# mbilos/stribor

Measured on NVIDIA B200. Metric: log_prob samples/s, 8-layer spline coupling d=64, higher is better.
Workload: dtype f32

## Files before the change

stribor_b200/csrc/tc_layer.cu:

```cuda
#include "common.cuh"
#include "stb_math.cuh"
#include "tc_common.cuh"
#include "tc_pack.cuh"
#include "tc_spline16.cuh"

namespace stb {
using namespace tc;

namespace tcl {
using namespace sp16;

constexpr int kHid = 64;
constexpr int kK1 = 32;
constexpr int kPPad = 48;
constexpr int kG = 2;
constexpr int kChunkN = kG * kPPad;
constexpr int kMaxDim = 64;
constexpr int kMaxTr = 32;
constexpr int kMaxChunks = kMaxTr / kG;
constexpr int kTileRows = 256;
constexpr int kXsStride = kMaxDim + 1;
constexpr int kStages = 3;
constexpr int kMaxChain = 8;
constexpr int kEpiPerSub = 2;
constexpr int kEpiWarps = 2 * 4 * kEpiPerSub;
constexpr int kEpiWarp0 = 3;
constexpr int kThreads = (kEpiWarp0 + kEpiWarps) * 32;
constexpr int kEpiThreads = kEpiWarps * 32;

constexpr uint32_t kMagic = 0x53544232u;
struct Header {
    uint32_t magic;
    int32_t kind, dim, n_cond, n_tr, n_chunks, P, act;
    float s2;
    uint32_t maxbits;
    int32_t cond_idx[kK1];
    int32_t tr_idx[kMaxTr];
    uint32_t noshift_mask;
    int32_t n_lat;
    int32_t n_bins;
    int32_t pad[256 - 13 - kK1 - kMaxTr];
};
static_assert(sizeof(Header) == 1024, "header layout");
constexpr uint32_t kOffB1 = 1024;
constexpr uint32_t kOffB2 = kOffB1 + kHid * 4;
constexpr uint32_t kSmallBytes = kOffB2 + kMaxChunks * kChunkN * 4;
constexpr uint32_t kOffW1 = 8192;
constexpr uint32_t kW1Part = kHid * kK1 * 2;
constexpr uint32_t kW1Bytes = 3 * kW1Part;
constexpr uint32_t kA1Part = 128 * kK1 * 2;
constexpr uint32_t kOffW2 = kOffW1 + kW1Bytes;
constexpr uint32_t kChunkBytes = 2 * kChunkN * kHid * 2;
constexpr uint32_t kPackedBytes = kOffW2 + kMaxChunks * kChunkBytes;
constexpr uint32_t kHeadBytes = kOffW1 + kW1Bytes;
static_assert(kHeadBytes <= kChunkBytes, "the layer head fits a ring stage");

constexpr uint32_t kSmXs = 0;
constexpr uint32_t kSmA = kSmXs + kTileRows * kXsStride * 4;
constexpr uint32_t kABytes = 32768;
constexpr uint32_t kSmW1 = kSmA + 2 * kABytes;
constexpr uint32_t kSmB = kSmW1 + kW1Bytes;
constexpr uint32_t kSmSmall = kSmB + kStages * kChunkBytes;
constexpr uint32_t kSmBar = (kSmSmall + kSmallBytes + 15) & ~15u;
constexpr uint32_t kSmLd = kSmBar + 256;
constexpr uint32_t kSmemBytes = kSmLd + (kEpiPerSub - 1) * kTileRows * 4;
static_assert(kSmemBytes <= 227 * 1024, "shared memory budget");
static_assert(kSmA % 16 == 0 && kSmW1 % 16 == 0 && kSmB % 16 == 0 && kSmSmall % 16 == 0, "alignment");

struct Bars {
    uint64_t acc_full[2][2], acc_empty[2][2];
    uint64_t setup;
    uint64_t b_full[kStages], b_empty[kStages];
    uint64_t a1_ready[2], acc1_full[2], h_ready[2];
};
static_assert(sizeof(Bars) <= 256, "barrier block");

constexpr uint32_t kColAcc1 = 0;
constexpr uint32_t kColAcc2 = 128;
constexpr uint32_t kTmemCols = 512;

struct Args {
    const uint8_t* packed;
    const float* x;
    float* y;
    float* ldj;
    int ldj_mode;
    int base_log_prob;
    int inverse;
    float lower, upper;
    long long rows;
    int n_tiles;
    int n_layers, dim;
    const uint8_t* chain_packed[kMaxChain];
    float lower_l[kMaxChain], upper_l[kMaxChain];
    int n_chunks_l[kMaxChain];
    const float* latent;
    int lat_stride;
    int32_t* bins;
    int permuted;
    ChainPerm perm;
};

template <int KIND, bool INVERSE, bool CHAIN, bool BINS = false>
__global__ void __launch_bounds__(kThreads, 1) tc_spline_layer_kernel(const Args A) {
    extern __shared__ __align__(1024) uint8_t smem[];
    float* xs = reinterpret_cast<float*>(smem + kSmXs);
    uint8_t* abuf = smem + kSmA;
    uint8_t* w1s = smem + kSmW1;
    uint8_t* bst = smem + kSmB;
    const Header* hdr = reinterpret_cast<const Header*>(smem + kSmSmall);
    const float* b1s = reinterpret_cast<const float*>(smem + kSmSmall + kOffB1);
    const float* b2s = reinterpret_cast<const float*>(smem + kSmSmall + kOffB2);
    Bars* bars = reinterpret_cast<Bars*>(smem + kSmBar);
    float* ld_s = reinterpret_cast<float*>(smem + kSmLd);

    const int tid = threadIdx.x, warp = tid >> 5, lane = tid & 31;

    if (tid == 0) {
        mbar_init(&bars->setup, 1);
        for (int i = 0; i < kStages; ++i) { mbar_init(&bars->b_full[i], 1); mbar_init(&bars->b_empty[i], 2); }
        for (int s = 0; s < 2; ++s) {
            mbar_init(&bars->a1_ready[s], kEpiWarps);
            mbar_init(&bars->acc1_full[s], 1);
            mbar_init(&bars->h_ready[s], kEpiWarps);
            for (int b = 0; b < 2; ++b) { mbar_init(&bars->acc_full[s][b], 1); mbar_init(&bars->acc_empty[s][b], 8); }
        }
        fence_mbar_init();
    }
    __shared__ uint32_t tmem_base_s;
    if (warp == 1) tmem_alloc(&tmem_base_s, kTmemCols);
    tc_fence_before();
    __syncthreads();
    tc_fence_after();
    const uint32_t tmem = tmem_base_s;

    if (!CHAIN) {
        if (tid == 0) {
            mbar_arrive_expect_tx(&bars->setup, kSmallBytes + kW1Bytes);
            bulk_g2s(smem + kSmSmall, A.packed, kSmallBytes, &bars->setup);
            bulk_g2s(w1s, A.packed + kOffW1, kW1Bytes, &bars->setup);
        }
        mbar_wait(&bars->setup, 0);
    }

    const int n_layers = CHAIN ? A.n_layers : 1;
    const int d = CHAIN ? A.dim : hdr->dim;
    int n_tr = CHAIN ? 0 : hdr->n_tr, n_cond = CHAIN ? 0 : hdr->n_cond, n_chunks = CHAIN ? 0 : hdr->n_chunks;
    int n_lat = CHAIN ? 0 : hdr->n_lat;
    int act = CHAIN ? 0 : hdr->act;
    float s2 = CHAIN ? 1.f : hdr->s2;
    float s2l = s2 * 1.4426950408889634f;
    const int dshift = ((d & (d - 1)) == 0) ? (31 - __clz(d)) : -1;
    const int my_tiles = (A.n_tiles > (int)blockIdx.x) ? (A.n_tiles - 1 - (int)blockIdx.x) / (int)gridDim.x + 1 : 0;

    if (warp == 0) {
        if (lane == 0) {
            uint32_t cc = 0;
            for (int it = 0; it < my_tiles; ++it) {
                if (it + 1 < my_tiles) {
                    const long long nrow0 = ((long long)blockIdx.x + (long long)(it + 1) * gridDim.x) * kTileRows;
                    const long long nb = min((long long)kTileRows, A.rows - nrow0) * d * 4;
                    const char* src = reinterpret_cast<const char*>(A.x + nrow0 * d);
                    if (nb >= 16 && ((reinterpret_cast<uintptr_t>(src) & 15) == 0))
                        asm volatile("cp.async.bulk.prefetch.L2.global [%0], %1;" ::"l"(src), "r"((uint32_t)(nb & ~15LL)) : "memory");
                }
                for (int l = 0; l < n_layers; ++l) {
                    const uint8_t* img = CHAIN ? A.chain_packed[l] : A.packed;
                    const int nch = CHAIN ? A.n_chunks_l[l] : n_chunks;
                    if (CHAIN) {
                        const uint32_t st = cc % kStages, use = cc / kStages;
                        mbar_wait_relaxed(&bars->b_empty[st], (use & 1) ^ 1);
                        mbar_arrive_expect_tx(&bars->b_full[st], kHeadBytes);
                        bulk_g2s(bst + st * kChunkBytes, img, kHeadBytes, &bars->b_full[st]);
                        ++cc;
                    }
                    for (int c = 0; c < nch; ++c, ++cc) {
                        const uint32_t st = cc % kStages, use = cc / kStages;
                        mbar_wait_relaxed(&bars->b_empty[st], (use & 1) ^ 1);
                        mbar_arrive_expect_tx(&bars->b_full[st], kChunkBytes);
                        bulk_g2s(bst + st * kChunkBytes, img + kOffW2 + (size_t)c * kChunkBytes, kChunkBytes,
                                 &bars->b_full[st]);
                    }
                }
            }
        }
    } else if (warp < kEpiWarp0) {
        if (lane == 0) {
            const int s = warp - 1;
            const uint32_t idesc1 = make_idesc(FMT_BF16, 128, kHid);
            const uint32_t idesc2 = make_idesc(FMT_F16, 128, kChunkN);
            uint32_t cc = 0;
            uint32_t rc = 0;
            uint32_t hp = 0;
            for (int it = 0; it < my_tiles; ++it)
            for (int l = 0; l < n_layers; ++l, ++hp) {
                const uint32_t tpar = hp & 1;
                const int nch = CHAIN ? A.n_chunks_l[l] : n_chunks;
                {
                    uint32_t b0 = smem_u32(w1s);
                    const uint32_t hst = rc % kStages;
                    if (CHAIN) {
                        mbar_wait_relaxed(&bars->b_full[hst], (rc / kStages) & 1);
                        b0 = smem_u32(bst + hst * kChunkBytes) + kOffW1;
                    }
                    mbar_wait_relaxed(&bars->a1_ready[s], tpar);
                    tc_fence_after();
                    const uint32_t a0 = smem_u32(abuf + s * kABytes);
                    const uint32_t dcol = tmem + kColAcc1 + s * kHid;
                    uint32_t acc = 0;
#pragma unroll
                    for (int p = 0; p < 8; ++p) {
                        const int pa = (p == 0 || p == 3 || p == 6) ? 1 : ((p == 1 || p == 4) ? 2 : 0);
                        const int pb = (p == 0 || p == 2) ? 2 : ((p == 1 || p == 3 || p == 5) ? 1 : 0);
#pragma unroll
                        for (int ks = 0; ks < kK1 / 16; ++ks) {
                            umma_f16(dcol, make_smem_desc(a0 + pa * kA1Part + ks * 256, 128, 512),
                                     make_smem_desc(b0 + pb * kW1Part + ks * 256, 128, 512), idesc1, acc);
                            acc = 1;
                        }
                    }
                    umma_commit(&bars->acc1_full[s]);
                    if (CHAIN) { umma_commit(&bars->b_empty[hst]); ++rc; }
                }
                for (int c = 0; c < nch; ++c, ++cc, ++rc) {
                    const uint32_t st = rc % kStages, use = rc / kStages;
                    mbar_wait_relaxed(&bars->b_full[st], use & 1);
                    const uint32_t buf = cc & 1, buse = cc >> 1;
                    if (c == 0) mbar_wait_relaxed(&bars->h_ready[s], tpar);
                    mbar_wait_relaxed(&bars->acc_empty[s][buf], (buse & 1) ^ 1);
                    tc_fence_after();
                    const uint32_t a_hi = smem_u32(abuf + s * kABytes), a_lo = a_hi + 16384;
                    const uint32_t b_hi = smem_u32(bst + st * kChunkBytes), b_lo = b_hi + 12288;
                    const uint32_t dcol = tmem + kColAcc2 + (s * 2 + buf) * kChunkN;
                    uint32_t acc = 0;
#pragma unroll
                    for (int p = 0; p < 3; ++p) {
                        const uint32_t aa = (p == 0) ? a_lo : a_hi, bb = (p == 1) ? b_lo : b_hi;
#pragma unroll
                        for (int ks = 0; ks < kHid / 16; ++ks) {
                            umma_f16(dcol, make_smem_desc(aa + ks * 256, 128, 1024),
                                     make_smem_desc(bb + ks * 256, 128, 1024), idesc2, acc);
                            acc = 1;
                        }
                    }
                    umma_commit(&bars->acc_full[s][buf]);
                    umma_commit(&bars->b_empty[st]);
                }
            }
        }
    } else if (warp >= kEpiWarp0) {
        const int q = warp & 3;
        const int cls = (warp - (kEpiWarp0 + ((q - kEpiWarp0) & 3))) >> 2;
        const int s = cls & 1, r3 = cls >> 1;
        const int etid = tid - kEpiWarp0 * 32;
        const int rloc = q * 32 + lane;
        const int rt = s * 128 + rloc;
        float* xrow = xs + rt * kXsStride;
        const uint32_t a_row_off = (uint32_t)(rloc >> 3) * 1024 + (uint32_t)(rloc & 7) * 16;
        const uint32_t lane_sel = (uint32_t)(q * 32) << 16;
        const bool want_ld = A.ldj_mode != STB_LDJ_NONE;
        float lo = A.lower, hi = A.upper;
        float inv_span = 1.f / (hi - lo);
        const uint32_t full_bar = pin(smem_u32(&bars->acc_full[s][0]));
        const uint32_t empty_bar = pin(smem_u32(&bars->acc_empty[s][0]));
        const uint32_t col_base = pin(tmem + lane_sel + kColAcc2 + (uint32_t)(s * 2) * kChunkN);
        const uint32_t tr_idx_a = pin(smem_u32(&hdr->tr_idx[0]));
        const uint32_t b2_a = pin(smem_u32(b2s));
        const uint32_t xrow_a = pin(smem_u32(xrow));
        uint32_t noshift_mask = CHAIN ? 0u : hdr->noshift_mask;
        uint32_t cc = 0, rc = 0, hp = 0;

        for (int it = 0; it < my_tiles; ++it) {
            const long long tile = (long long)blockIdx.x + (long long)it * gridDim.x;
            const long long row0 = tile * kTileRows;
            const int nrows = (int)min((long long)kTileRows, A.rows - row0);

            {
                const float* xg = A.x + row0 * d;
                const int n = nrows * d;
                if ((d & 3) == 0 && ((reinterpret_cast<uintptr_t>(xg) & 15) == 0)) {
                    const int n4 = (kTileRows * d) >> 2;
                    for (int i0 = etid; i0 < n4; i0 += kEpiThreads * 4) {
                        float4 v[4];
#pragma unroll
                        for (int u = 0; u < 4; ++u) {
                            const int i = i0 + u * kEpiThreads;
                            v[u] = (i < n4 && i * 4 < n) ? __ldg(reinterpret_cast<const float4*>(xg) + i)
                                                         : make_float4(0.f, 0.f, 0.f, 0.f);
                        }
#pragma unroll
                        for (int u = 0; u < 4; ++u) {
                            const int i = i0 + u * kEpiThreads;
                            if (i < n4) {
                                const int r = (dshift >= 0) ? ((i * 4) >> dshift) : (i * 4) / d, c = (i * 4) - r * d;
                                float* dst = xs + r * kXsStride + c;
                                dst[0] = v[u].x; dst[1] = v[u].y; dst[2] = v[u].z; dst[3] = v[u].w;
                            }
                        }
                    }
                } else {
                    for (int i = etid; i < kTileRows * d; i += kEpiThreads) {
                        const int r = i / d, c = i - r * d;
                        xs[r * kXsStride + c] = (i < n) ? __ldg(xg + i) : 0.f;
                    }
                }
            }
            named_bar_sync(1, kEpiThreads);
            float ld_acc = 0.f;
#pragma unroll 1
            for (int l = 0; l < n_layers; ++l, ++hp) {
            const uint32_t tpar = hp & 1;
            if (CHAIN) {
                const uint32_t hst = rc % kStages;
                mbar_wait(&bars->b_full[hst], (rc / kStages) & 1);
                const uint4* src = reinterpret_cast<const uint4*>(bst + hst * kChunkBytes);
                uint4* dst = reinterpret_cast<uint4*>(smem + kSmSmall);
                for (int i = etid; i < (int)(kSmallBytes / 16); i += kEpiThreads) dst[i] = src[i];
                named_bar_sync(1, kEpiThreads);
                if (A.permuted) {
                    Header* h = const_cast<Header*>(hdr);
                    if (etid < kK1) { if (etid < h->n_cond) h->cond_idx[etid] = A.perm.phys[l][h->cond_idx[etid]]; }
                    else if (etid < kK1 + kMaxTr) h->tr_idx[etid - kK1] = A.perm.phys[l][h->tr_idx[etid - kK1]];
                    named_bar_sync(1, kEpiThreads);
                }
                n_tr = hdr->n_tr; n_cond = hdr->n_cond; n_chunks = hdr->n_chunks; act = hdr->act;
                n_lat = hdr->n_lat;
                s2 = hdr->s2; s2l = s2 * 1.4426950408889634f;
                noshift_mask = hdr->noshift_mask;
                lo = A.lower_l[l]; hi = A.upper_l[l]; inv_span = 1.f / (hi - lo);
                asm volatile("" : "+f"(lo), "+f"(hi), "+f"(inv_span));
                rc += 1u + (uint32_t)n_chunks;
            }

#pragma unroll 1
            for (int sp = 0; sp < 2; ++sp) {
                const float* xr = xs + (sp * 128 + rloc) * kXsStride;
                uint8_t* a_p = abuf + sp * kABytes;
                const uint32_t a1_row_off = (uint32_t)(rloc >> 3) * 512 + (uint32_t)(rloc & 7) * 16;
#pragma unroll 1
                for (int kc = cls; kc < kK1 / 8; kc += 2 * kEpiPerSub) {
                    __align__(16) __nv_bfloat16 q0[8], q1[8], q2[8];
#pragma unroll
                    for (int u = 0; u < 8; ++u) {
                        const int k = kc * 8 + u;
                        float v = 0.f;
                        if (k < n_cond) v = xr[hdr->cond_idx[k]];
                        else if (k < n_cond + n_lat && sp * 128 + rloc < nrows)
                            v = __ldg(A.latent + (row0 + sp * 128 + rloc) * A.lat_stride + (k - n_cond));
                        split_bf16x3(v, q0[u], q1[u], q2[u]);
                    }
                    *reinterpret_cast<uint4*>(a_p + a1_row_off + kc * 128) = *reinterpret_cast<const uint4*>(q0);
                    *reinterpret_cast<uint4*>(a_p + kA1Part + a1_row_off + kc * 128) = *reinterpret_cast<const uint4*>(q1);
                    *reinterpret_cast<uint4*>(a_p + 2 * kA1Part + a1_row_off + kc * 128) = *reinterpret_cast<const uint4*>(q2);
                }
                fence_proxy_async_smem();
                __syncwarp();
                if (lane == 0) mbar_arrive(&bars->a1_ready[sp]);
            }
#pragma unroll 1
            for (int sp = 0; sp < 2; ++sp) {
                uint8_t* a_p = abuf + sp * kABytes;
                mbar_wait(&bars->acc1_full[sp], tpar);
                tc_fence_after();
#pragma unroll 1
                for (int kc = cls; kc < kHid / 8; kc += 2 * kEpiPerSub) {
                    const int c0 = kc * 8;
                    float v[8];
                    tmem_ld8(tmem + lane_sel + kColAcc1 + sp * kHid + c0, v);
                    tmem_ld_wait();
                    __align__(16) __half hh[8], hl[8];
                    if (act == STB_ACT_TANH) {
#pragma unroll
                        for (int i = 0; i < 8; ++i) split_f16(tanh_fast(v[i] + b1s[c0 + i]), hh[i], hl[i]);
                    } else {
#pragma unroll
                        for (int i = 0; i < 8; ++i) v[i] = sigmoid_act(v[i] + b1s[c0 + i]);
#pragma unroll
                        for (int i = 0; i < 8; ++i) split_f16(v[i], hh[i], hl[i]);
                    }
                    *reinterpret_cast<uint4*>(a_p + a_row_off + kc * 128) = *reinterpret_cast<const uint4*>(hh);
                    *reinterpret_cast<uint4*>(a_p + 16384 + a_row_off + kc * 128) = *reinterpret_cast<const uint4*>(hl);
                }
                tc_fence_before();
                fence_proxy_async_smem();
                __syncwarp();
                if (lane == 0) mbar_arrive(&bars->h_ready[sp]);
            }

#pragma unroll 1
            for (int ji = r3; ji < kG * n_chunks; ji += kEpiPerSub) {
                const uint32_t ccc = cc + (uint32_t)(ji >> 1);
                const uint32_t buf = ccc & 1, buse = ccc >> 1;
                const int g = ji & 1;
                uint32_t j4;
                asm volatile("ld.shared.u32 %0, [%1];" : "=r"(j4) : "r"(tr_idx_a + 4u * (uint32_t)(ji < n_tr ? ji : 0)));
                j4 <<= 2;
                float xv;
                asm volatile("ld.shared.f32 %0, [%1];" : "=f"(xv) : "r"(xrow_a + j4));
                const bool inside = (ji < n_tr) && (xv >= lo) && (xv <= hi);
                const float* bb = b2s + ji * kPPad;
                mbar_wait_a(full_bar + buf * 8, buse & 1);
                tc_fence_after();
                const uint32_t col0 = col_base + buf * kChunkN + (uint32_t)g * kPPad;
                float out = xv, ld = 0.f;
                const bool shift = !((noshift_mask >> (ji & 31)) & 1u);
                const float2* bb2 = reinterpret_cast<const float2*>(bb);
                if (KIND == STB_RQS) {
                    RqsLoc loc;
                    {
                        float2 t[kBins];
                        tmem_ld16(col0, reinterpret_cast<float*>(t));
                        tmem_ld16(col0 + 16, reinterpret_cast<float*>(t) + 16);
                        tmem_ld_wait();
#pragma unroll
                        for (int i = 0; i < kBins; ++i) t[i] = __ffma2_rn(t[i], f2(s2l), bb2[i]);
                        loc = rqs16_locate<INVERSE>(t, shift, lo, inv_span, xv);
                    }
                    float dd[16];
                    tmem_ld16(col0 + 2 * kBins, dd);
                    tmem_ld_wait();
                    tc_fence_before();
                    __syncwarp();
                    if (lane == 0) mbar_arrive_a(empty_bar + buf * 8);
                    if (inside) {
                        float r0, r1;
                        pick_pair16(dd, loc.k, r0, r1);
                        const float u0 = (loc.k == 0) ? STB_RQS_EDGE_CONST : fmaf(r0, s2, bb[2 * kBins + loc.k - 1]);
                        const float u1 = (loc.k == kBins - 1) ? STB_RQS_EDGE_CONST : fmaf(r1, s2, bb[2 * kBins + loc.k]);
                        rqs16_finish<INVERSE>(loc, u0, u1, lo, hi, want_ld, xv, out, ld);
                    }
                    if (BINS && ji < n_tr && rt < nrows) A.bins[(row0 + rt) * d + (j4 >> 2)] = inside ? loc.k : -1;
                } else {
                    const float span = hi - lo;
                    const float u = (xv - lo) / span;
                    CubSel sel;
                    {
                        float2 t[kBins];
                        tmem_ld16(col0, reinterpret_cast<float*>(t));
                        tmem_ld16(col0 + 16, reinterpret_cast<float*>(t) + 16);
                        tmem_ld_wait();
#pragma unroll
                        for (int i = 0; i < kBins; ++i) t[i] = __ffma2_rn(t[i], f2(s2l), bb2[i]);
                        sel = cubic16_locate<INVERSE>(t, shift, u);
                    }
                    float dd[8];
                    tmem_ld8(col0 + 2 * kBins, dd);
                    tmem_ld_wait();
                    tc_fence_before();
                    __syncwarp();
                    if (lane == 0) mbar_arrive_a(empty_bar + buf * 8);
                    if (inside) {
                        const float ul = fmaf(dd[0], s2, bb[2 * kBins]), ur = fmaf(dd[1], s2, bb[2 * kBins + 1]);
                        cubic16_finish<INVERSE>(sel, ul, ur, lo, hi, want_ld, u, out, ld);
                    }
                    if (BINS && ji < n_tr && rt < nrows) A.bins[(row0 + rt) * d + (j4 >> 2)] = inside ? sel.k : -1;
                }
                if (ji < n_tr) asm volatile("st.shared.f32 [%0], %1;" ::"r"(xrow_a + j4), "f"(out) : "memory");
                ld_acc += ld;
            }
            cc += (uint32_t)n_chunks;
            if (CHAIN && l + 1 < n_layers) named_bar_sync(1, kEpiThreads);
            }

            if (r3 < kEpiPerSub - 1) ld_s[r3 * kTileRows + rt] = ld_acc;
            named_bar_sync(1, kEpiThreads);
            if (r3 == kEpiPerSub - 1 && want_ld && rt < nrows) {
                float tot = ld_s[rt];
#pragma unroll
                for (int o = 1; o < kEpiPerSub - 1; ++o) tot += ld_s[o * kTileRows + rt];
                tot += ld_acc;
                if (A.base_log_prob) {
                    float b = 0.f;
                    for (int c = 0; c < d; ++c) { const float v = xrow[c]; b += -0.5f * v * v - 0.91893853320467274178f; }
                    tot += b;
                }
                float* dst = A.ldj + row0 + rt;
                *dst = (A.ldj_mode == STB_LDJ_ADD) ? (*dst + tot) : tot;
            }

            if (A.y != nullptr) {
                float* yg = A.y + row0 * d;
                const int n = nrows * d;
                if (CHAIN && A.permuted) {
                    for (int i = etid; i < n; i += kEpiThreads) {
                        const int r = (dshift >= 0) ? (i >> dshift) : i / d, c = i - r * d;
                        yg[i] = xs[r * kXsStride + A.perm.out_phys[c]];
                    }
                } else if ((d & 3) == 0 && ((reinterpret_cast<uintptr_t>(yg) & 15) == 0)) {
                    const int n4 = n >> 2;
                    for (int i = etid; i < n4; i += kEpiThreads) {
                        const int r = (dshift >= 0) ? ((i * 4) >> dshift) : (i * 4) / d, c = (i * 4) - r * d;
                        const float* src = xs + r * kXsStride + c;
                        reinterpret_cast<float4*>(yg)[i] = make_float4(src[0], src[1], src[2], src[3]);
                    }
                } else {
                    for (int i = etid; i < n; i += kEpiThreads) {
                        const int r = i / d, c = i - r * d;
                        yg[i] = xs[r * kXsStride + c];
                    }
                }
            }
            named_bar_sync(1, kEpiThreads);
        }
    }

    tc_fence_before();
    __syncthreads();
    if (warp == 1) tmem_dealloc(tmem, kTmemCols);
}

constexpr int kPRows = 128;
constexpr int kPEpiWarp0 = 2;
constexpr int kPEpiWarps = 8;
constexpr int kPThreads = (kPEpiWarp0 + kPEpiWarps) * 32;
constexpr int kPEpiThreads = kPEpiWarps * 32;
constexpr uint32_t kPSmXs = 0;
constexpr uint32_t kPSmB = kPRows * kXsStride * 4;
constexpr uint32_t kPSmSmall = kPSmB + kStages * kChunkBytes;
constexpr uint32_t kPSmBar = (kPSmSmall + kSmallBytes + 15) & ~15u;
constexpr uint32_t kPSmemBytes = kPSmBar + 256;
static_assert(kPSmB % 128 == 0 && kPSmSmall % 16 == 0, "alignment");
static_assert(2 * (kPSmemBytes + 1024) <= 228 * 1024, "two CTAs per SM");
struct PBars {
    uint64_t acc_full[2], acc_empty[2];
    uint64_t b_full[kStages], b_empty[kStages];
    uint64_t a1_ready, acc1_full, h_ready;
    uint32_t tmem_base;
};
static_assert(sizeof(PBars) <= 256, "barrier block");
constexpr uint32_t kPColH = 0;
constexpr uint32_t kPColAcc = kHid;
constexpr uint32_t kPColA1 = kPColAcc + kChunkN;
constexpr uint32_t kPTmemCols = 256;

__device__ __forceinline__ void tmem_st4(uint32_t taddr, const uint32_t* r) {
    asm volatile("tcgen05.st.sync.aligned.32x32b.x4.b32 [%0], {%1, %2, %3, %4};" ::"r"(taddr), "r"(r[0]), "r"(r[1]),
// ... 350 lines not shown
    if (warp == 1) tmem_dealloc(tmem, kPTmemCols);
}

struct PackLayout {
    using Hdr = Header;
    static constexpr uint32_t kMagic = tcl::kMagic, kOffB1 = tcl::kOffB1, kOffW1 = tcl::kOffW1;
    static constexpr int kK1 = tcl::kK1, kMaxTr = tcl::kMaxTr;
    static __device__ void header_extra(Header*, const SplinePackArgs&) {}
};

static_assert(kMaxTr == kK1, "spline_gate bounds the transformed dims by GEMM1's K");
static bool admit(const stb_layer* L, MaskSplit& m) {
    return spline_gate(L, kMaxDim, kK1, m) && L->net.n_linear == 2 && L->net.dims[1] == kHid;
}

}

bool tc_layer_supported(const stb_layer* L) {
    tcl::MaskSplit m;
    return tcl::admit(L, m);
}

uint64_t tc_packed_bytes(const stb_layer*) { return tcl::kPackedBytes; }

int tc_pack_layer(const stb_layer* L, void* out, cudaStream_t stream) {
    using namespace tcl;
    SplinePackArgs a;
    if (!admit(L, a.m)) return set_error(STB_ENOTSUP, "layer has no tensor-core path");
    a.out = static_cast<uint8_t*>(out);
    a.n_chunks = (a.m.n_tr + kG - 1) / kG;
    a.n_lat = L->latent_dim; a.n_bins = L->n_bins;
    a.kind = L->kind; a.dim = L->dim; a.P = spline_params_per_dim(L->kind, L->n_bins);
    a.act = L->net.activation;
    a.W1 = L->net.W[0]; a.b1 = L->net.b[0]; a.W2 = L->net.W[1]; a.b2 = L->net.b[1];
    const BoundArgs b = spline_bound_args(a.m, a.W2, a.b2, kHid, a.P, a.n_bins, a.act,
                                          a.out + offsetof(Header, noshift_mask));
    return pack_image(out, sizeof(Header), stream, "tc_pack", [&] {
        pack_pass(spline64_maxabs_kernel<PackLayout>, 64, 256, stream, a);
        pack_pass(spline64_pack_kernel<PackLayout>, 296, 256, stream, a);
        pack_pass(tc_bound_kernel, 1, kMaxTr * 32, stream, b);
    });
}

namespace tcl {
static int launch_pair(Args& A, int kind, bool full, int64_t rows, cudaStream_t stream) {
    void (*kern)(Args) = pick_variant(kind, A.inverse, full, [](auto K, auto I, auto F) { return tc_spline_pair_kernel<K, I, F>; });
    const long long ptiles = (rows + kPRows - 1) / kPRows;
    if (ptiles > 0x7fffffffLL) return set_error(STB_EINVAL, "too many rows");
    A.n_tiles = (int)ptiles;
    const cudaError_t pe = cudaFuncSetAttribute(kern, cudaFuncAttributePreferredSharedMemoryCarveout, 100);
    if (pe != cudaSuccess) return set_error(STB_ECUDA, "cudaFuncSetAttribute: %s", cudaGetErrorString(pe));
    return launch_persistent(kern, A, ptiles, 2, kPThreads, kPSmemBytes, stream, "tc_spline_pair_kernel");
}
}

int tc_layer_apply(const stb_layer* L, int direction, const float* x, const float* latent, float* y, float* ldj,
                   int ldj_mode, int base_log_prob, int64_t rows, cudaStream_t stream, int32_t* bins) {
    using namespace tcl;
    if (L->packed_bytes < kPackedBytes) return set_error(STB_EINVAL, "packed image too small");
    Args A = {};
    A.bins = bins;
    A.latent = L->latent_dim > 0 ? latent : nullptr;
    A.lat_stride = L->latent_dim;
    if (L->n_bins != kBins) {
        if (bins) return set_error(STB_ENOTSUP, "the bin-index instrument of the tensor-core path covers 16-bin layers");
        MaskSplit m;
        if (!admit(L, m)) return set_error(STB_EINVAL, "layer has no tensor-core path");
        A.x = x; A.y = y; A.ldj = ldj;
        A.ldj_mode = ldj ? ldj_mode : STB_LDJ_NONE;
        A.base_log_prob = base_log_prob;
        A.inverse = direction == STB_INVERSE;
        A.rows = rows;
        A.n_layers = 1; A.dim = L->dim;
        A.chain_packed[0] = static_cast<const uint8_t*>(L->packed);
        A.lower_l[0] = L->lower; A.upper_l[0] = L->upper;
        A.n_chunks_l[0] = (m.n_tr + kG - 1) / kG;
        return launch_pair(A, L->kind, false, rows, stream);
    }
    A.packed = static_cast<const uint8_t*>(L->packed);
    A.x = x; A.y = y; A.ldj = ldj;
    A.ldj_mode = ldj ? ldj_mode : STB_LDJ_NONE;
    A.base_log_prob = base_log_prob;
    A.inverse = direction == STB_INVERSE;
    A.lower = L->lower; A.upper = L->upper;
    A.rows = rows;
    const long long tiles = (rows + kTileRows - 1) / kTileRows;
    if (tiles > 0x7fffffffLL) return set_error(STB_EINVAL, "too many rows");
    A.n_tiles = (int)tiles;

    void (*kern)(Args) = pick_variant(L->kind, A.inverse, bins != nullptr,
                                      [](auto K, auto I, auto B) { return tc_spline_layer_kernel<K, I, false, B>; });
    return launch_persistent(kern, A, tiles, 1, kThreads, kSmemBytes, stream, "tc_spline_layer_kernel");
}


bool tc_chain_supported(const stb_layer* const* layers, int n) {
    using namespace tcl;
    if (n < 2 || n > kMaxChain) return false;
    for (int i = 0; i < n; ++i) {
        const stb_layer* L = layers[i];
        if (!L->packed || L->packed_bytes < kPackedBytes || !tc_layer_supported(L)) return false;
        if (L->kind != layers[0]->kind || L->dim != layers[0]->dim) return false;
        if (L->latent_dim != layers[0]->latent_dim) return false;
    }
    return true;
}

int tc_chain_apply(const stb_layer* const* layers, int n, int direction, const float* x, const float* latent, float* y,
                   float* ldj, int ldj_mode, int base_log_prob, int64_t rows, cudaStream_t stream, const ChainPerm* perm) {
    using namespace tcl;
    if (!tc_chain_supported(layers, n)) return set_error(STB_EINVAL, "layers cannot be chained");
    Args A = {};
    A.latent = layers[0]->latent_dim > 0 ? latent : nullptr;
    A.lat_stride = layers[0]->latent_dim;
    if (A.lat_stride > 0 && !latent) return set_error(STB_EINVAL, "layer expects a latent input");
    if (perm) { A.permuted = 1; A.perm = *perm; }
    A.packed = static_cast<const uint8_t*>(layers[0]->packed);
    A.x = x; A.y = y; A.ldj = ldj;
    A.ldj_mode = ldj ? ldj_mode : STB_LDJ_NONE;
    A.base_log_prob = base_log_prob;
    A.inverse = direction == STB_INVERSE;
    A.lower = layers[0]->lower; A.upper = layers[0]->upper;
    A.rows = rows;
    A.n_layers = n;
    A.dim = layers[0]->dim;
    for (int i = 0; i < n; ++i) {
        MaskSplit m;
        if (!admit(layers[i], m)) return set_error(STB_EINVAL, "layer has no tensor-core path");
        A.chain_packed[i] = static_cast<const uint8_t*>(layers[i]->packed);
        A.lower_l[i] = layers[i]->lower; A.upper_l[i] = layers[i]->upper;
        A.n_chunks_l[i] = (m.n_tr + kG - 1) / kG;
    }
    const long long tiles = (rows + kTileRows - 1) / kTileRows;
    if (tiles > 0x7fffffffLL) return set_error(STB_EINVAL, "too many rows");
    A.n_tiles = (int)tiles;
    bool full = true;
    for (int i = 0; i < n; ++i) full = full && layers[i]->n_bins == kBins;
    const bool use_pair = !full || tiles < (long long)sm_count();
    if (use_pair) return launch_pair(A, layers[0]->kind, full, rows, stream);
    void (*kern)(Args) = pick_variant(layers[0]->kind, A.inverse, [](auto K, auto I) { return tc_spline_layer_kernel<K, I, true>; });
    return launch_persistent(kern, A, tiles, 1, kThreads, kSmemBytes, stream, "tc_spline_layer_kernel (chain)");
}

}
```

Baseline: 166.4 million.

## Keep hidden activations in TMEM and write next-layer A1 inputs from the epilogue

The second GEMM now takes the hidden activations directly from tensor memory (TS-form MMA) instead of staging them in a shared-memory A buffer. The layer head is split out: small header data goes through a double-buffered ring and W1 through its own barrier pair, so the old per-layer copy into shared memory goes away. Host-built tables (conditioner columns, transform columns, next-layer A1 slots) are copied into shared memory. The epilogue writes each transformed output straight into the next layer's A1 operand, so only the missing conditioners are rebuilt early. Subtile halves also sync independently. Together these aim to remove the shared-memory round trip, the header copy and the full epilogue barriers between layers, at the cost of more complex barrier logic and a larger kernel-argument struct.

Result: faster. 172.0 million (median of 6 runs) (+3.3%).

```diff
diff --git a/stribor_b200/csrc/tc_layer.cu b/stribor_b200/csrc/tc_layer.cu
--- a/stribor_b200/csrc/tc_layer.cu
+++ b/stribor_b200/csrc/tc_layer.cu
@@ -55,22 +55,34 @@
 constexpr uint32_t kHeadBytes = kOffW1 + kW1Bytes;
 static_assert(kHeadBytes <= kChunkBytes, "the layer head fits a ring stage");
 
+struct LayerTabs {
+    uint8_t tr_col[kMaxChain][kMaxTr];
+    uint8_t cond_col[kMaxChain][kK1];
+    int16_t next_a1[kMaxChain][kMaxTr];
+    uint32_t a1_early[kMaxChain];
+    int32_t n_cond[kMaxChain];
+};
+static_assert(sizeof(LayerTabs) % 16 == 0, "copied as uint4");
+
 constexpr uint32_t kSmXs = 0;
-constexpr uint32_t kSmA = kSmXs + kTileRows * kXsStride * 4;
-constexpr uint32_t kABytes = 32768;
-constexpr uint32_t kSmW1 = kSmA + 2 * kABytes;
+constexpr uint32_t kSmA1 = kSmXs + kTileRows * kXsStride * 4;
+constexpr uint32_t kA1Sub = 3 * kA1Part;
+constexpr uint32_t kSmW1 = kSmA1 + 2 * kA1Sub;
 constexpr uint32_t kSmB = kSmW1 + kW1Bytes;
 constexpr uint32_t kSmSmall = kSmB + kStages * kChunkBytes;
-constexpr uint32_t kSmBar = (kSmSmall + kSmallBytes + 15) & ~15u;
-constexpr uint32_t kSmLd = kSmBar + 256;
+constexpr uint32_t kSmBar = (kSmSmall + 2 * kSmallBytes + 15) & ~15u;
+constexpr uint32_t kSmTab = kSmBar + 256;
+constexpr uint32_t kSmLd = kSmTab + sizeof(LayerTabs);
 constexpr uint32_t kSmemBytes = kSmLd + (kEpiPerSub - 1) * kTileRows * 4;
 static_assert(kSmemBytes <= 227 * 1024, "shared memory budget");
-static_assert(kSmA % 16 == 0 && kSmW1 % 16 == 0 && kSmB % 16 == 0 && kSmSmall % 16 == 0, "alignment");
+static_assert(kSmA1 % 16 == 0 && kSmW1 % 16 == 0 && kSmB % 16 == 0 && kSmSmall % 16 == 0 && kSmallBytes % 16 == 0 &&
+              kSmTab % 16 == 0, "alignment");
 
 struct Bars {
     uint64_t acc_full[2][2], acc_empty[2][2];
-    uint64_t setup;
     uint64_t b_full[kStages], b_empty[kStages];
+    uint64_t w1_full, w1_empty;
+    uint64_t small_full[2], small_empty[2];
     uint64_t a1_ready[2], acc1_full[2], h_ready[2];
 };
 static_assert(sizeof(Bars) <= 256, "barrier block");
@@ -80,14 +92,12 @@
 constexpr uint32_t kTmemCols = 512;
 
 struct Args {
-    const uint8_t* packed;
     const float* x;
     float* y;
     float* ldj;
     int ldj_mode;
     int base_log_prob;
     int inverse;
-    float lower, upper;
     long long rows;
     int n_tiles;
     int n_layers, dim;
@@ -99,34 +109,37 @@
     int32_t* bins;
     int permuted;
     ChainPerm perm;
+    LayerTabs tab;
 };
 
-template <int KIND, bool INVERSE, bool CHAIN, bool BINS = false>
+template <int KIND, bool INVERSE, bool BINS = false>
 __global__ void __launch_bounds__(kThreads, 1) tc_spline_layer_kernel(const Args A) {
     extern __shared__ __align__(1024) uint8_t smem[];
     float* xs = reinterpret_cast<float*>(smem + kSmXs);
-    uint8_t* abuf = smem + kSmA;
     uint8_t* w1s = smem + kSmW1;
     uint8_t* bst = smem + kSmB;
-    const Header* hdr = reinterpret_cast<const Header*>(smem + kSmSmall);
-    const float* b1s = reinterpret_cast<const float*>(smem + kSmSmall + kOffB1);
-    const float* b2s = reinterpret_cast<const float*>(smem + kSmSmall + kOffB2);
     Bars* bars = reinterpret_cast<Bars*>(smem + kSmBar);
+    LayerTabs* tab = reinterpret_cast<LayerTabs*>(smem + kSmTab);
     float* ld_s = reinterpret_cast<float*>(smem + kSmLd);
 
     const int tid = threadIdx.x, warp = tid >> 5, lane = tid & 31;
 
     if (tid == 0) {
-        mbar_init(&bars->setup, 1);
         for (int i = 0; i < kStages; ++i) { mbar_init(&bars->b_full[i], 1); mbar_init(&bars->b_empty[i], 2); }
+        mbar_init(&bars->w1_full, 1);
+        mbar_init(&bars->w1_empty, 2);
         for (int s = 0; s < 2; ++s) {
-            mbar_init(&bars->a1_ready[s], kEpiWarps);
+            mbar_init(&bars->small_full[s], 1);
+            mbar_init(&bars->small_empty[s], kEpiWarps);
+            mbar_init(&bars->a1_ready[s], kEpiWarps / 2);
             mbar_init(&bars->acc1_full[s], 1);
-            mbar_init(&bars->h_ready[s], kEpiWarps);
+            mbar_init(&bars->h_ready[s], kEpiWarps / 2);
             for (int b = 0; b < 2; ++b) { mbar_init(&bars->acc_full[s][b], 1); mbar_init(&bars->acc_empty[s][b], 8); }
         }
         fence_mbar_init();
     }
+    for (int i = tid; i < (int)(sizeof(LayerTabs) / 16); i += kThreads)
+        reinterpret_cast<uint4*>(tab)[i] = reinterpret_cast<const uint4*>(&A.tab)[i];
     __shared__ uint32_t tmem_base_s;
     if (warp == 1) tmem_alloc(&tmem_base_s, kTmemCols);
     tc_fence_before();
@@ -134,28 +147,14 @@
     tc_fence_after();
     const uint32_t tmem = tmem_base_s;
 
-    if (!CHAIN) {
-        if (tid == 0) {
-            mbar_arrive_expect_tx(&bars->setup, kSmallBytes + kW1Bytes);
-            bulk_g2s(smem + kSmSmall, A.packed, kSmallBytes, &bars->setup);
-            bulk_g2s(w1s, A.packed + kOffW1, kW1Bytes, &bars->setup);
-        }
-        mbar_wait(&bars->setup, 0);
-    }
-
-    const int n_layers = CHAIN ? A.n_layers : 1;
-    const int d = CHAIN ? A.dim : hdr->dim;
-    int n_tr = CHAIN ? 0 : hdr->n_tr, n_cond = CHAIN ? 0 : hdr->n_cond, n_chunks = CHAIN ? 0 : hdr->n_chunks;
-    int n_lat = CHAIN ? 0 : hdr->n_lat;
-    int act = CHAIN ? 0 : hdr->act;
-    float s2 = CHAIN ? 1.f : hdr->s2;
-    float s2l = s2 * 1.4426950408889634f;
+    const int n_layers = A.n_layers;
+    const int d = A.dim;
     const int dshift = ((d & (d - 1)) == 0) ? (31 - __clz(d)) : -1;
     const int my_tiles = (A.n_tiles > (int)blockIdx.x) ? (A.n_tiles - 1 - (int)blockIdx.x) / (int)gridDim.x + 1 : 0;
 
     if (warp == 0) {
         if (lane == 0) {
-            uint32_t cc = 0;
+            uint32_t cc = 0, hp = 0;
             for (int it = 0; it < my_tiles; ++it) {
                 if (it + 1 < my_tiles) {
                     const long long nrow0 = ((long long)blockIdx.x + (long long)(it + 1) * gridDim.x) * kTileRows;
@@ -164,17 +163,16 @@
                     if (nb >= 16 && ((reinterpret_cast<uintptr_t>(src) & 15) == 0))
                         asm volatile("cp.async.bulk.prefetch.L2.global [%0], %1;" ::"l"(src), "r"((uint32_t)(nb & ~15LL)) : "memory");
                 }
-                for (int l = 0; l < n_layers; ++l) {
-                    const uint8_t* img = CHAIN ? A.chain_packed[l] : A.packed;
-                    const int nch = CHAIN ? A.n_chunks_l[l] : n_chunks;
-                    if (CHAIN) {
-                        const uint32_t st = cc % kStages, use = cc / kStages;
-                        mbar_wait_relaxed(&bars->b_empty[st], (use & 1) ^ 1);
-                        mbar_arrive_expect_tx(&bars->b_full[st], kHeadBytes);
-                        bulk_g2s(bst + st * kChunkBytes, img, kHeadBytes, &bars->b_full[st]);
-                        ++cc;
-                    }
-                    for (int c = 0; c < nch; ++c, ++cc) {
+                for (int l = 0; l < n_layers; ++l, ++hp) {
+                    const uint8_t* img = A.chain_packed[l];
+                    const uint32_t sb = hp & 1;
+                    mbar_wait_relaxed(&bars->small_empty[sb], ((hp >> 1) & 1) ^ 1);
+                    mbar_arrive_expect_tx(&bars->small_full[sb], kSmallBytes);
+                    bulk_g2s(smem + kSmSmall + sb * kSmallBytes, img, kSmallBytes, &bars->small_full[sb]);
+                    mbar_wait_relaxed(&bars->w1_empty, (hp & 1) ^ 1);
+                    mbar_arrive_expect_tx(&bars->w1_full, kW1Bytes);
+                    bulk_g2s(w1s, img + kOffW1, kW1Bytes, &bars->w1_full);
+                    for (int c = 0; c < A.n_chunks_l[l]; ++c, ++cc) {
                         const uint32_t st = cc % kStages, use = cc / kStages;
                         mbar_wait_relaxed(&bars->b_empty[st], (use & 1) ^ 1);
                         mbar_arrive_expect_tx(&bars->b_full[st], kChunkBytes);
@@ -189,24 +187,18 @@
             const int s = warp - 1;
             const uint32_t idesc1 = make_idesc(FMT_BF16, 128, kHid);
             const uint32_t idesc2 = make_idesc(FMT_F16, 128, kChunkN);
+            const uint32_t hcol = tmem + kColAcc1 + s * kHid;
             uint32_t cc = 0;
-            uint32_t rc = 0;
             uint32_t hp = 0;
             for (int it = 0; it < my_tiles; ++it)
             for (int l = 0; l < n_layers; ++l, ++hp) {
                 const uint32_t tpar = hp & 1;
-                const int nch = CHAIN ? A.n_chunks_l[l] : n_chunks;
+                const int nch = A.n_chunks_l[l];
                 {
-                    uint32_t b0 = smem_u32(w1s);
-                    const uint32_t hst = rc % kStages;
-                    if (CHAIN) {
-                        mbar_wait_relaxed(&bars->b_full[hst], (rc / kStages) & 1);
-                        b0 = smem_u32(bst + hst * kChunkBytes) + kOffW1;
-                    }
+                    mbar_wait_relaxed(&bars->w1_full, tpar);
                     mbar_wait_relaxed(&bars->a1_ready[s], tpar);
                     tc_fence_after();
-                    const uint32_t a0 = smem_u32(abuf + s * kABytes);
-                    const uint32_t dcol = tmem + kColAcc1 + s * kHid;
+                    const uint32_t a0 = smem_u32(smem + kSmA1 + s * kA1Sub), b0 = smem_u32(w1s);
                     uint32_t acc = 0;
 #pragma unroll
                     for (int p = 0; p < 8; ++p) {
@@ -214,32 +206,30 @@
                         const int pb = (p == 0 || p == 2) ? 2 : ((p == 1 || p == 3 || p == 5) ? 1 : 0);
 #pragma unroll
                         for (int ks = 0; ks < kK1 / 16; ++ks) {
-                            umma_f16(dcol, make_smem_desc(a0 + pa * kA1Part + ks * 256, 128, 512),
+                            umma_f16(hcol, make_smem_desc(a0 + pa * kA1Part + ks * 256, 128, 512),
                                      make_smem_desc(b0 + pb * kW1Part + ks * 256, 128, 512), idesc1, acc);
                             acc = 1;
                         }
                     }
                     umma_commit(&bars->acc1_full[s]);
-                    if (CHAIN) { umma_commit(&bars->b_empty[hst]); ++rc; }
-                }
-                for (int c = 0; c < nch; ++c, ++cc, ++rc) {
-                    const uint32_t st = rc % kStages, use = rc / kStages;
+                    umma_commit(&bars->w1_empty);
+                }
+                for (int c = 0; c < nch; ++c, ++cc) {
+                    const uint32_t st = cc % kStages, use = cc / kStages;
                     mbar_wait_relaxed(&bars->b_full[st], use & 1);
                     const uint32_t buf = cc & 1, buse = cc >> 1;
                     if (c == 0) mbar_wait_relaxed(&bars->h_ready[s], tpar);
                     mbar_wait_relaxed(&bars->acc_empty[s][buf], (buse & 1) ^ 1);
                     tc_fence_after();
-                    const uint32_t a_hi = smem_u32(abuf + s * kABytes), a_lo = a_hi + 16384;
                     const uint32_t b_hi = smem_u32(bst + st * kChunkBytes), b_lo = b_hi + 12288;
                     const uint32_t dcol = tmem + kColAcc2 + (s * 2 + buf) * kChunkN;
                     uint32_t acc = 0;
 #pragma unroll
                     for (int p = 0; p < 3; ++p) {
-                        const uint32_t aa = (p == 0) ? a_lo : a_hi, bb = (p == 1) ? b_lo : b_hi;
+                        const uint32_t a_off = (p == 0) ? 8u : 0u, bb = (p == 1) ? b_lo : b_hi;
 #pragma unroll
                         for (int ks = 0; ks < kHid / 16; ++ks) {
-                            umma_f16(dcol, make_smem_desc(aa + ks * 256, 128, 1024),
-                                     make_smem_desc(bb + ks * 256, 128, 1024), idesc2, acc);
+                            umma_f16_ts(dcol, hcol + ks * 16 + a_off, make_smem_desc(bb + ks * 256, 128, 1024), idesc2, acc);
                             acc = 1;
                         }
                     }
@@ -256,19 +246,49 @@
         const int rloc = q * 32 + lane;
         const int rt = s * 128 + rloc;
         float* xrow = xs + rt * kXsStride;
-        const uint32_t a_row_off = (uint32_t)(rloc >> 3) * 1024 + (uint32_t)(rloc & 7) * 16;
+        uint8_t* a1row = smem + kSmA1 + s * kA1Sub + (rloc >> 3) * 512 + (rloc & 7) * 16;
         const uint32_t lane_sel = (uint32_t)(q * 32) << 16;
         const bool want_ld = A.ldj_mode != STB_LDJ_NONE;
-        float lo = A.lower, hi = A.upper;
-        float inv_span = 1.f / (hi - lo);
         const uint32_t full_bar = pin(smem_u32(&bars->acc_full[s][0]));
         const uint32_t empty_bar = pin(smem_u32(&bars->acc_empty[s][0]));
         const uint32_t col_base = pin(tmem + lane_sel + kColAcc2 + (uint32_t)(s * 2) * kChunkN);
-        const uint32_t tr_idx_a = pin(smem_u32(&hdr->tr_idx[0]));
-        const uint32_t b2_a = pin(smem_u32(b2s));
         const uint32_t xrow_a = pin(smem_u32(xrow));
-        uint32_t noshift_mask = CHAIN ? 0u : hdr->noshift_mask;
-        uint32_t cc = 0, rc = 0, hp = 0;
+        const uint32_t a1row_a = pin(smem_u32(a1row));
+        const int n_lat = A.latent ? A.lat_stride : 0;
+        uint32_t cc = 0, hp = 0;
+
+        auto write_a1_early = [&](int L, long long row0, int nrows) {
+            const uint32_t bits = tab->a1_early[L];
+            const int nc = tab->n_cond[L];
+#pragma unroll 1
+            for (int kc = r3; kc < kK1 / 8; kc += 2) {
+                const uint32_t gbits = (bits >> (kc * 8)) & 0xffu;
+                if (gbits == 0) continue;
+                __align__(16) __nv_bfloat16 q0[8], q1[8], q2[8];
+#pragma unroll
+                for (int u = 0; u < 8; ++u) {
+                    const int k = kc * 8 + u;
+                    float v = 0.f;
+                    if (k < nc) v = xrow[tab->cond_col[L][k]];
+                    else if (k < nc + n_lat && rt < nrows) v = __ldg(A.latent + (row0 + rt) * A.lat_stride + (k - nc));
+                    split_bf16x3(v, q0[u], q1[u], q2[u]);
+                }
+                uint8_t* dst = a1row + kc * 128;
+                if (gbits == 0xffu) {
+                    *reinterpret_cast<uint4*>(dst) = *reinterpret_cast<const uint4*>(q0);
+                    *reinterpret_cast<uint4*>(dst + kA1Part) = *reinterpret_cast<const uint4*>(q1);
+                    *reinterpret_cast<uint4*>(dst + 2 * kA1Part) = *reinterpret_cast<const uint4*>(q2);
+                } else {
+#pragma unroll
+                    for (int u = 0; u < 8; ++u) {
+                        if (!((gbits >> u) & 1u)) continue;
+                        reinterpret_cast<__nv_bfloat16*>(dst)[u] = q0[u];
+                        reinterpret_cast<__nv_bfloat16*>(dst + kA1Part)[u] = q1[u];
+                        reinterpret_cast<__nv_bfloat16*>(dst + 2 * kA1Part)[u] = q2[u];
+                    }
+                }
+            }
+        };
 
         for (int it = 0; it < my_tiles; ++it) {
             const long long tile = (long long)blockIdx.x + (long long)it * gridDim.x;
@@ -306,86 +326,55 @@
                 }
             }
             named_bar_sync(1, kEpiThreads);
+            write_a1_early(0, row0, nrows);
+            fence_proxy_async_smem();
+            __syncwarp();
+            if (lane == 0) mbar_arrive(&bars->a1_ready[s]);
             float ld_acc = 0.f;
 #pragma unroll 1
             for (int l = 0; l < n_layers; ++l, ++hp) {
-            const uint32_t tpar = hp & 1;
-            if (CHAIN) {
-                const uint32_t hst = rc % kStages;
-                mbar_wait(&bars->b_full[hst], (rc / kStages) & 1);
-                const uint4* src = reinterpret_cast<const uint4*>(bst + hst * kChunkBytes);
-                uint4* dst = reinterpret_cast<uint4*>(smem + kSmSmall);
-                for (int i = etid; i < (int)(kSmallBytes / 16); i += kEpiThreads) dst[i] = src[i];
-                named_bar_sync(1, kEpiThreads);
-                if (A.permuted) {
-                    Header* h = const_cast<Header*>(hdr);
-                    if (etid < kK1) { if (etid < h->n_cond) h->cond_idx[etid] = A.perm.phys[l][h->cond_idx[etid]]; }
-                    else if (etid < kK1 + kMaxTr) h->tr_idx[etid - kK1] = A.perm.phys[l][h->tr_idx[etid - kK1]];
-                    named_bar_sync(1, kEpiThreads);
-                }
-                n_tr = hdr->n_tr; n_cond = hdr->n_cond; n_chunks = hdr->n_chunks; act = hdr->act;
-                n_lat = hdr->n_lat;
-                s2 = hdr->s2; s2l = s2 * 1.4426950408889634f;
-                noshift_mask = hdr->noshift_mask;
-                lo = A.lower_l[l]; hi = A.upper_l[l]; inv_span = 1.f / (hi - lo);
-                asm volatile("" : "+f"(lo), "+f"(hi), "+f"(inv_span));
-                rc += 1u + (uint32_t)n_chunks;
-            }
-
-#pragma unroll 1
-            for (int sp = 0; sp < 2; ++sp) {
-                const float* xr = xs + (sp * 128 + rloc) * kXsStride;
-                uint8_t* a_p = abuf + sp * kABytes;
-                const uint32_t a1_row_off = (uint32_t)(rloc >> 3) * 512 + (uint32_t)(rloc & 7) * 16;
-#pragma unroll 1
-                for (int kc = cls; kc < kK1 / 8; kc += 2 * kEpiPerSub) {
-                    __align__(16) __nv_bfloat16 q0[8], q1[8], q2[8];
-#pragma unroll
-                    for (int u = 0; u < 8; ++u) {
-                        const int k = kc * 8 + u;
-                        float v = 0.f;
-                        if (k < n_cond) v = xr[hdr->cond_idx[k]];
-                        else if (k < n_cond + n_lat && sp * 128 + rloc < nrows)
-                            v = __ldg(A.latent + (row0 + sp * 128 + rloc) * A.lat_stride + (k - n_cond));
-                        split_bf16x3(v, q0[u], q1[u], q2[u]);
-                    }
-                    *reinterpret_cast<uint4*>(a_p + a1_row_off + kc * 128) = *reinterpret_cast<const uint4*>(q0);
-                    *reinterpret_cast<uint4*>(a_p + kA1Part + a1_row_off + kc * 128) = *reinterpret_cast<const uint4*>(q1);
-                    *reinterpret_cast<uint4*>(a_p + 2 * kA1Part + a1_row_off + kc * 128) = *reinterpret_cast<const uint4*>(q2);
-                }
-                fence_proxy_async_smem();
-                __syncwarp();
-                if (lane == 0) mbar_arrive(&bars->a1_ready[sp]);
-            }
-#pragma unroll 1
-            for (int sp = 0; sp < 2; ++sp) {
-                uint8_t* a_p = abuf + sp * kABytes;
-                mbar_wait(&bars->acc1_full[sp], tpar);
-                tc_fence_after();
-#pragma unroll 1
-                for (int kc = cls; kc < kHid / 8; kc += 2 * kEpiPerSub) {
-                    const int c0 = kc * 8;
-                    float v[8];
-                    tmem_ld8(tmem + lane_sel + kColAcc1 + sp * kHid + c0, v);
-                    tmem_ld_wait();
-                    __align__(16) __half hh[8], hl[8];
-                    if (act == STB_ACT_TANH) {
-#pragma unroll
-                        for (int i = 0; i < 8; ++i) split_f16(tanh_fast(v[i] + b1s[c0 + i]), hh[i], hl[i]);
-                    } else {
-#pragma unroll
-                        for (int i = 0; i < 8; ++i) v[i] = sigmoid_act(v[i] + b1s[c0 + i]);
-#pragma unroll
-                        for (int i = 0; i < 8; ++i) split_f16(v[i], hh[i], hl[i]);
-                    }
-                    *reinterpret_cast<uint4*>(a_p + a_row_off + kc * 128) = *reinterpret_cast<const uint4*>(hh);
-                    *reinterpret_cast<uint4*>(a_p + 16384 + a_row_off + kc * 128) = *reinterpret_cast<const uint4*>(hl);
-                }
-                tc_fence_before();
-                fence_proxy_async_smem();
-                __syncwarp();
-                if (lane == 0) mbar_arrive(&bars->h_ready[sp]);
-            }
+            const uint32_t tpar = hp & 1, sb = hp & 1;
+            const uint8_t* small = smem + kSmSmall + sb * kSmallBytes;
+            const Header* hdr = reinterpret_cast<const Header*>(small);
+            const float* b1s = reinterpret_cast<const float*>(small + kOffB1);
+            const float* b2s = reinterpret_cast<const float*>(small + kOffB2);
+            mbar_wait(&bars->small_full[sb], (hp >> 1) & 1);
+            const int n_tr = hdr->n_tr, n_chunks = hdr->n_chunks, act = hdr->act;
+            const float s2 = hdr->s2, s2l = s2 * 1.4426950408889634f;
+            const uint32_t noshift_mask = hdr->noshift_mask;
+            float lo = A.lower_l[l], hi = A.upper_l[l], inv_span = 1.f / (hi - lo);
+            asm volatile("" : "+f"(lo), "+f"(hi), "+f"(inv_span));
+            const uint32_t tr_a = pin(smem_u32(&tab->tr_col[l][0]));
+            const uint32_t nx_a = pin(smem_u32(&tab->next_a1[l][0]));
+
+            mbar_wait(&bars->acc1_full[s], tpar);
+            tc_fence_after();
+            float vh[2][16];
+            tmem_ld16(tmem + lane_sel + kColAcc1 + s * kHid + r3 * 32, vh[0]);
+            tmem_ld16(tmem + lane_sel + kColAcc1 + s * kHid + r3 * 32 + 16, vh[1]);
+            tmem_ld_wait();
+#pragma unroll
+            for (int blk = 0; blk < 2; ++blk) {
+                const int c0 = r3 * 32 + blk * 16;
+                const float* v = vh[blk];
+                uint32_t hh[8], hl[8];
+                if (act == STB_ACT_TANH) {
+#pragma unroll
+                    for (int i = 0; i < 8; ++i)
+                        split_f16x2_sat(tanh_fast(v[2 * i] + b1s[c0 + 2 * i]), tanh_fast(v[2 * i + 1] + b1s[c0 + 2 * i + 1]), hh[i], hl[i]);
+                } else {
+#pragma unroll
+                    for (int i = 0; i < 8; ++i)
+                        split_f16x2_sat(sigmoid_act(v[2 * i] + b1s[c0 + 2 * i]), sigmoid_act(v[2 * i + 1] + b1s[c0 + 2 * i + 1]), hh[i], hl[i]);
+                }
+                tmem_st8(tmem + lane_sel + kColAcc1 + s * kHid + c0, hh);
+                tmem_st8(tmem + lane_sel + kColAcc1 + s * kHid + c0 + 8, hl);
+            }
+            tmem_st_wait();
+            tc_fence_before();
+            __syncwarp();
+            if (lane == 0) mbar_arrive(&bars->h_ready[s]);
+            if (l + 1 < n_layers) write_a1_early(l + 1, row0, nrows);
 
 #pragma unroll 1
             for (int ji = r3; ji < kG * n_chunks; ji += kEpiPerSub) {
@@ -393,7 +382,7 @@
                 const uint32_t buf = ccc & 1, buse = ccc >> 1;
                 const int g = ji & 1;
                 uint32_t j4;
-                asm volatile("ld.shared.u32 %0, [%1];" : "=r"(j4) : "r"(tr_idx_a + 4u * (uint32_t)(ji < n_tr ? ji : 0)));
+                asm volatile("ld.shared.u8 %0, [%1];" : "=r"(j4) : "r"(tr_a + (uint32_t)ji));
                 j4 <<= 2;
                 float xv;
                 asm volatile("ld.shared.f32 %0, [%1];" : "=f"(xv) : "r"(xrow_a + j4));
@@ -456,10 +445,29 @@
                     if (BINS && ji < n_tr && rt < nrows) A.bins[(row0 + rt) * d + (j4 >> 2)] = inside ? sel.k : -1;
                 }
                 if (ji < n_tr) asm volatile("st.shared.f32 [%0], %1;" ::"r"(xrow_a + j4), "f"(out) : "memory");
+                int nx;
+                asm volatile("ld.shared.s16 %0, [%1];" : "=r"(nx) : "r"(nx_a + 2u * (uint32_t)ji));
+                if (nx >= 0) {
+                    __nv_bfloat16 q0, q1, q2;
+                    split_bf16x3(out, q0, q1, q2);
+                    const uint32_t a = a1row_a + (uint32_t)nx;
+                    asm volatile("st.shared.b16 [%0], %1;" ::"r"(a), "h"(__bfloat16_as_ushort(q0)) : "memory");
+                    asm volatile("st.shared.b16 [%0], %1;" ::"r"(a + kA1Part), "h"(__bfloat16_as_ushort(q1)) : "memory");
+                    asm volatile("st.shared.b16 [%0], %1;" ::"r"(a + 2 * kA1Part), "h"(__bfloat16_as_ushort(q2)) : "memory");
+                }
                 ld_acc += ld;
             }
             cc += (uint32_t)n_chunks;
-            if (CHAIN && l + 1 < n_layers) named_bar_sync(1, kEpiThreads);
+            if (l + 1 < n_layers) fence_proxy_async_smem();
+            __syncwarp();
+            if (lane == 0) {
+                mbar_arrive(&bars->small_empty[sb]);
+                if (l + 1 < n_layers) mbar_arrive(&bars->a1_ready[s]);
+            }
+            if (l + 1 < n_layers) {
+                if (s == 0) asm volatile("bar.sync 2, %0;" ::"n"(kEpiThreads / 2) : "memory");
+                else asm volatile("bar.sync 3, %0;" ::"n"(kEpiThreads / 2) : "memory");
+            }
             }
 
             if (r3 < kEpiPerSub - 1) ld_s[r3 * kTileRows + rt] = ld_acc;
@@ -481,7 +489,7 @@
             if (A.y != nullptr) {
                 float* yg = A.y + row0 * d;
                 const int n = nrows * d;
-                if (CHAIN && A.permuted) {
+                if (A.permuted) {
                     for (int i = etid; i < n; i += kEpiThreads) {
                         const int r = (dshift >= 0) ? (i >> dshift) : i / d, c = i - r * d;
                         yg[i] = xs[r * kXsStride + A.perm.out_phys[c]];
@@ -938,6 +946,41 @@
     if (pe != cudaSuccess) return set_error(STB_ECUDA, "cudaFuncSetAttribute: %s", cudaGetErrorString(pe));
     return launch_persistent(kern, A, ptiles, 2, kPThreads, kPSmemBytes, stream, "tc_spline_pair_kernel");
 }
+
+static int set_layers(Args& A, const stb_layer* const* layers, int n, const ChainPerm* perm) {
+    A.n_layers = n;
+    A.dim = layers[0]->dim;
+    if (perm) { A.permuted = 1; A.perm = *perm; }
+    MaskSplit m[kMaxChain];
+    for (int l = 0; l < n; ++l) {
+        if (!admit(layers[l], m[l])) return set_error(STB_EINVAL, "layer has no tensor-core path");
+        A.chain_packed[l] = static_cast<const uint8_t*>(layers[l]->packed);
+        A.lower_l[l] = layers[l]->lower; A.upper_l[l] = layers[l]->upper;
+        A.n_chunks_l[l] = (m[l].n_tr + kG - 1) / kG;
+    }
+    LayerTabs& T = A.tab;
+    const auto col = [&](int l, int c) { return (uint8_t)(perm ? perm->phys[l][c] : c); };
+    for (int l = 0; l < n; ++l) {
+        T.n_cond[l] = m[l].n_cond;
+        for (int k = 0; k < kK1; ++k) T.cond_col[l][k] = k < m[l].n_cond ? col(l, m[l].cond_idx[k]) : 0;
+        for (int ji = 0; ji < kMaxTr; ++ji) T.tr_col[l][ji] = col(l, m[l].tr_idx[ji]);
+    }
+    for (int l = 0; l < n; ++l) {
+        uint32_t produced = 0;
+        for (int ji = 0; ji < kMaxTr; ++ji) {
+            T.next_a1[l][ji] = -1;
+            if (l + 1 == n || ji >= m[l].n_tr) continue;
+            for (int k = 0; k < m[l + 1].n_cond; ++k)
+                if (T.cond_col[l + 1][k] == T.tr_col[l][ji]) {
+                    T.next_a1[l][ji] = (int16_t)((k / 8) * 128 + (k % 8) * 2);
+                    produced |= 1u << k;
+                }
+        }
+        if (l + 1 < n) T.a1_early[l + 1] = ~produced;
+    }
+    T.a1_early[0] = ~0u;
+    return STB_OK;
+}
 }
 
 int tc_layer_apply(const stb_layer* L, int direction, const float* x, const float* latent, float* y, float* ldj,
@@ -948,34 +991,23 @@
     A.bins = bins;
     A.latent = L->latent_dim > 0 ? latent : nullptr;
     A.lat_stride = L->latent_dim;
-    if (L->n_bins != kBins) {
-        if (bins) return set_error(STB_ENOTSUP, "the bin-index instrument of the tensor-core path covers 16-bin layers");
-        MaskSplit m;
-        if (!admit(L, m)) return set_error(STB_EINVAL, "layer has no tensor-core path");
-        A.x = x; A.y = y; A.ldj = ldj;
-        A.ldj_mode = ldj ? ldj_mode : STB_LDJ_NONE;
-        A.base_log_prob = base_log_prob;
-        A.inverse = direction == STB_INVERSE;
-        A.rows = rows;
-        A.n_layers = 1; A.dim = L->dim;
-        A.chain_packed[0] = static_cast<const uint8_t*>(L->packed);
-        A.lower_l[0] = L->lower; A.upper_l[0] = L->upper;
-        A.n_chunks_l[0] = (m.n_tr + kG - 1) / kG;
-        return launch_pair(A, L->kind, false, rows, stream);
-    }
-    A.packed = static_cast<const uint8_t*>(L->packed);
     A.x = x; A.y = y; A.ldj = ldj;
     A.ldj_mode = ldj ? ldj_mode : STB_LDJ_NONE;
     A.base_log_prob = base_log_prob;
     A.inverse = direction == STB_INVERSE;
-    A.lower = L->lower; A.upper = L->upper;
     A.rows = rows;
+    const int rc = set_layers(A, &L, 1, nullptr);
+    if (rc != STB_OK) return rc;
+    if (L->n_bins != kBins) {
+        if (bins) return set_error(STB_ENOTSUP, "the bin-index instrument of the tensor-core path covers 16-bin layers");
+        return launch_pair(A, L->kind, false, rows, stream);
+    }
     const long long tiles = (rows + kTileRows - 1) / kTileRows;
     if (tiles > 0x7fffffffLL) return set_error(STB_EINVAL, "too many rows");
     A.n_tiles = (int)tiles;
 
     void (*kern)(Args) = pick_variant(L->kind, A.inverse, bins != nullptr,
-                                      [](auto K, auto I, auto B) { return tc_spline_layer_kernel<K, I, false, B>; });
+                                      [](auto K, auto I, auto B) { return tc_spline_layer_kernel<K, I, B>; });
     return launch_persistent(kern, A, tiles, 1, kThreads, kSmemBytes, stream, "tc_spline_layer_kernel");
 }
 
@@ -1000,23 +1032,13 @@
     A.latent = layers[0]->latent_dim > 0 ? latent : nullptr;
     A.lat_stride = layers[0]->latent_dim;
     if (A.lat_stride > 0 && !latent) return set_error(STB_EINVAL, "layer expects a latent input");
-    if (perm) { A.permuted = 1; A.perm = *perm; }
-    A.packed = static_cast<const uint8_t*>(layers[0]->packed);
     A.x = x; A.y = y; A.ldj = ldj;
     A.ldj_mode = ldj ? ldj_mode : STB_LDJ_NONE;
     A.base_log_prob = base_log_prob;
     A.inverse = direction == STB_INVERSE;
-    A.lower = layers[0]->lower; A.upper = layers[0]->upper;
     A.rows = rows;
-    A.n_layers = n;
-    A.dim = layers[0]->dim;
-    for (int i = 0; i < n; ++i) {
-        MaskSplit m;
-        if (!admit(layers[i], m)) return set_error(STB_EINVAL, "layer has no tensor-core path");
-        A.chain_packed[i] = static_cast<const uint8_t*>(layers[i]->packed);
-        A.lower_l[i] = layers[i]->lower; A.upper_l[i] = layers[i]->upper;
-        A.n_chunks_l[i] = (m.n_tr + kG - 1) / kG;
-    }
+    const int rc = set_layers(A, layers, n, perm);
+    if (rc != STB_OK) return rc;
     const long long tiles = (rows + kTileRows - 1) / kTileRows;
     if (tiles > 0x7fffffffLL) return set_error(STB_EINVAL, "too many rows");
     A.n_tiles = (int)tiles;
@@ -1024,7 +1046,7 @@
     for (int i = 0; i < n; ++i) full = full && layers[i]->n_bins == kBins;
     const bool use_pair = !full || tiles < (long long)sm_count();
     if (use_pair) return launch_pair(A, layers[0]->kind, full, rows, stream);
-    void (*kern)(Args) = pick_variant(layers[0]->kind, A.inverse, [](auto K, auto I) { return tc_spline_layer_kernel<K, I, true>; });
+    void (*kern)(Args) = pick_variant(layers[0]->kind, A.inverse, [](auto K, auto I) { return tc_spline_layer_kernel<K, I>; });
     return launch_persistent(kern, A, tiles, 1, kThreads, kSmemBytes, stream, "tc_spline_layer_kernel (chain)");
 }
 
```
